# cristianpjensen/thesis-pai-reconstruction

Measured on NVIDIA B200. Metric: pix2pix_gan_train_images_per_sec_256x256, higher is better.
Workload: dtype bf16

## Files before the change

### thesis-pai-reconstruction_b200/csrc/igemm.cu

```cuda
#include <stdio.h>
#include <stdlib.h>

#include "pai_common.cuh"
#include "pai_epilogue.cuh"
#include "pai_kernels.h"

namespace pai {

#ifdef PAI_PROFILE_ROLES
#define ROLE_T0() const long long _t0 = clock64()
#define ROLE_ADD(var) var += clock64() - _t0
#else
#define ROLE_T0()
#define ROLE_ADD(var)
#endif

static constexpr int kThreads = 256;
static constexpr int kFpropThreads = 384;
static constexpr int kMaxStages = 8;

struct __align__(8) PipeSmem {
    uint64_t full[kMaxStages];
    uint64_t empty[kMaxStages];
    uint64_t acc_full[2];
// ... 315 lines not shown
            }
        };
        auto flush_stats = [&]() {
            if (st_col < 0) return;
            reduce_add(st_sum, st_sq, st_col);
#pragma unroll
            for (int j = 0; j < 8; ++j) st_sum[j] = st_sq[j] = 0.f;
            st_col = -1;
        };
        int it = 0;
        for (int t = worker; t < total_tiles; t += workers, ++it) {
            int nt, rr, mt, phase_idx, tw, th, tn;
            const int tt = p.fd_splitk.quot(t);
            p.fd_n_tiles.divmod(tt, rr, nt);
            p.fd_m_tiles.divmod(rr, phase_idx, mt);
            if (PAIR) mt = 2 * mt + (int)rank;
            p.fd_tiles_w.divmod(mt, mt, tw);
            p.fd_tiles_h.divmod(mt, tn, th);
            const int col0 = nt * n_tile;
            const int gw = tw * p.bw + (rpos & 255), gh = th * p.bh + ((rpos >> 8) & 255), gn = tn * p.bn + (rpos >> 16);
            const bool row_ok = (gw < p.gw) && (gh < p.gh) && (gn < p.gn);
            const int a = it & 1;
            const uint32_t acc_phase = (it >> 1) & 1;
            const bool fast = p.tma_out && (n_tile & 63) == 0 && col0 + n_tile <= p.cout &&
                              (p.bias == nullptr || (reinterpret_cast<uintptr_t>(p.bias) & 15) == 0);
            const int bw0 = tw * p.bw + (qpos & 255), bh0 = th * p.bh + ((qpos >> 8) & 255), bn0 = tn * p.bn + (qpos >> 16);
            const bool masked = MASKED && p.mask_src != nullptr && fast;
            auto mask_load = [&](int c) {
                __syncwarp();
                if (lane == 0) {
                    bulk_wait_group_read0();
                    mbar_expect_tx(&ps.mask_full[warp - 4], 32 * 128);
                    tma_load_4d(tile, &om.aux[fused ? c >> 6 : phase_idx], &ps.mask_full[warp - 4], col0 + (fused ? 0 : c),
                                bw0, bh0, bn0);
                }
            };
            if (masked && 64 * half < acc_n) mask_load(64 * half);
            {
                ROLE_T0();
                mbar_wait(&ps.acc_full[a], acc_phase);
                ROLE_ADD(prof_wait);
            }
#ifdef PAI_PROFILE_ROLES
            const long long twork = clock64();
#endif
            tc_fence_after();
            const uint32_t tmem_d = tmem_base + a * acc_cols + ((uint32_t)(q * 32) << 16);
// ... 64 lines not shown
                                if ((rows_ok >> row) & 1u) {
                                    const uint4 val = tile[row * 8 + (ch ^ (row & 7))];
                                    const __nv_bfloat162* hv = reinterpret_cast<const __nv_bfloat162*>(&val);
#pragma unroll
                                    for (int j = 0; j < 4; ++j) {
                                        const float2 f = __bfloat1622float2(hv[j]);
                                        cs[2 * j] += f.x;
                                        cs[2 * j + 1] += f.y;
                                        cq[2 * j] = fmaf(f.x, f.x, cq[2 * j]);
                                        cq[2 * j + 1] = fmaf(f.y, f.y, cq[2 * j + 1]);
                                    }
                                }
                            }
                            if (st_persist) {
#pragma unroll
                                for (int j = 0; j < 8; ++j) st_sum[j] += cs[j], st_sq[j] += cq[j];
                            } else {
                                reduce_add(cs, cq, col0 + oc);
                            }
                        }
                        if (masked && c + 128 < acc_n) mask_load(c + 128);
                    }
                }
            } else {
                const long long off = p.out_phase_off[phase_idx] + (long long)gn * p.out_sn + (long long)gh * p.out_sh +
                                      (long long)gw * p.out_sw + col0;
                const long long off2 = (long long)gn * p.out2_sn + (long long)gh * p.out2_sh + (long long)gw * p.out2_sw + col0;
                const bool vec_ok = ((p.cout & 7) == 0) && ((off & 7) == 0) && ((off2 & 7) == 0);
                int step = 0;
                for (int cc = 0; cc < n_tile; cc += 16, ++step) {
                    if ((step & 1) != half) continue;
                    uint32_t v[16];
                    __syncwarp();
                    tmem_ld_16(tmem_d + (uint32_t)cc, v);
                    tmem_ld_wait();
                    if (!row_ok || col0 + cc >= p.cout) continue;
                    float f[16];
#pragma unroll
                    for (int j = 0; j < 16; ++j) {
                        float x = __uint_as_float(v[j]);
                        if (p.bias != nullptr && col0 + cc + j < p.cout) x += __ldg(p.bias + col0 + cc + j);
                        f[j] = x;
                    }
                    if (p.accumulate) {
                        float* o = reinterpret_cast<float*>(p.out) + off + cc;
                        if (col0 + cc + 16 <= p.cout && ((off + cc) & 3) == 0) {
// ... 32 lines not shown
        if (p.bn_part != nullptr) flush_stats();
        if (lane == 0) bulk_wait_group0();
#ifdef PAI_PROFILE_ROLES
        if (blockIdx.x == 0 && threadIdx.x == 128)
            printf("[roles] epilogue warp 4: waiting for a full accumulator %lld cyc, working %lld cyc over %d tiles\n", prof_wait, prof_total, it);
#endif
    }
    tc_fence_before();
    if (PAIR)
        cluster_sync_all();
    else
        __syncthreads();
    if (warp == 2) {
        tc_fence_after();
        if (PAIR)
            tmem_dealloc_pair(tmem_base, 2 * acc_cols);
        else
            tmem_dealloc(tmem_base, 2 * acc_cols);
    }
}

__global__ void __launch_bounds__(kThreads, 1)
igemm_wgrad_kernel(const __grid_constant__ CUtensorMap tm_u, const __grid_constant__ CUtensorMap tm_s,
                   const IgemmWgradParams p) {
    pdl_launch_dependents();
    extern __shared__ uint8_t smem_raw[];
    __shared__ PipeSmem ps;
    uint8_t* smem = reinterpret_cast<uint8_t*>((reinterpret_cast<uintptr_t>(smem_raw) + 1023) & ~uintptr_t(1023));

    const int warp = threadIdx.x >> 5, lane = threadIdx.x & 31;
    const int mb = p.mb, nbt = p.nbt;
    const uint32_t blk_bytes = 64 * 128;
    const uint32_t a_bytes = 2 * mb * blk_bytes;
    const uint32_t stage_bytes = a_bytes + nbt * blk_bytes;
    const int stages = p.stages;
    const int n_cols = nbt * 64;
    const uint32_t tmem_cols = tmem_cols_for(mb * 256);

    const long long units = (long long)p.tiles * p.kblocks;
    const long long u_begin = units * blockIdx.x / gridDim.x, u_end = units * (blockIdx.x + 1) / gridDim.x;

    if (warp == 0 && lane == 0) {
        tma_prefetch_desc(&tm_u);
        tma_prefetch_desc(&tm_s);
    }
    if (warp == 1 && lane == 0) {
        for (int s = 0; s < stages; ++s) {
            mbar_init(&ps.full[s], 1);
            mbar_init(&ps.empty[s], 1);
        }
// ... 74 lines not shown
                    }
                }
                umma_commit(&ps.acc_full[0]);
                ++seg;
            }
        }
    } else if (warp >= 4) {
        const int q = warp & 3;
        const int r = q * 32 + lane;
        int seg = 0;
        long long u = u_begin;
        while (u < u_end) {
            const int tile = (int)(u / p.kblocks);
            const long long tile_end = (long long)(tile + 1) * p.kblocks;
            u = tile_end < u_end ? tile_end : u_end;
            const int ng = tile % p.n_groups, cu0 = (tile / p.n_groups) * 128 * mb;
            mbar_wait(&ps.acc_full[0], seg & 1);
            tc_fence_after();
            for (int a = 0; a < mb; ++a) {
                const int row = cu0 + a * 128 + r;
                const bool row_ok = row < p.cu;
                for (int nb = 0; nb < nbt; ++nb) {
                    const int blk = ng * nbt + nb, tap = blk / p.cs_blocks, cb = blk - tap * p.cs_blocks;
                    float* o = p.out + ((size_t)tap * p.cu + row) * (size_t)p.cs + cb * 64;
#pragma unroll
                    for (int c = 0; c < 64; c += 16) {
                        uint32_t v[16];
                        __syncwarp();
                        tmem_ld_16(tmem_base + ((uint32_t)(q * 32) << 16) + (uint32_t)(a * 256 + nb * 64 + c), v);
                        tmem_ld_wait();
                        if (row_ok) {
#pragma unroll
                            for (int j = 0; j < 16; j += 4)
                                red_add_v4(o + c + j, __uint_as_float(v[j]), __uint_as_float(v[j + 1]),
                                           __uint_as_float(v[j + 2]), __uint_as_float(v[j + 3]));
                        }
                    }
                }
            }
            tc_fence_before();
            __syncwarp();
            if (lane == 0) mbar_arrive_relaxed(&ps.acc_empty[0]);
            ++seg;
        }
    }
    tc_fence_before();
    __syncthreads();
    if (warp == 2) {
        tc_fence_after();
        tmem_dealloc(tmem_base, tmem_cols);
    }
}

static int pick_stages(size_t stage_bytes, size_t budget) {
    int s = (int)(budget / stage_bytes);
    if (s > kMaxStages) s = kMaxStages;
    if (s < 2) s = 2;
    return s;
}

bool igemm_fprop_use_pair(int n_tile, long long m_tiles, int n_tiles, int phases, int splitk) {
    static const bool off = getenv("PAI_NO_CTA_PAIR") != nullptr;
    if (off || splitk > 1 || n_tile % 32 != 0) return false;
    return ((m_tiles + 1) / 2) * n_tiles * phases >= 74;
}

int launch_igemm_fprop(const CUtensorMap& tm_a, const CUtensorMap& tm_b, const IgemmOutMaps& om, IgemmFpropParams p,
// ... 82 lines not shown
        const int c = (int)(i - pix * cout);
        float v = ws[i];
        if (bias != nullptr) v += bias[c];
        v = apply_act(v, act, slope);
        if (y_f32)
            reinterpret_cast<float*>(y)[pix * y_ld + c] = v;
        else
            reinterpret_cast<__nv_bfloat16*>(y)[pix * y_ld + c] = __float2bfloat16_rn(v);
    }
}

int launch_splitk_finish(const float* ws, long long pixels, int cout, const float* bias, int act, float slope, void* y,
                         int y_ld, int y_f32, cudaStream_t stream) {
    const long long total = pixels * cout;
    long long blocks = (total + 255) / 256;
    const int sms = sm_count(current_device());
    if (sms < 0) return -1;
    if (blocks > sms * 8) blocks = sms * 8;
    PAI_CUDA_OK(launch_pdl(splitk_finish_kernel, dim3((unsigned)blocks), dim3(256), 0, stream, 1, ws, total, cout, bias, act, slope, y, y_ld, y_f32));
    PAI_CUDA_OK(cudaGetLastError());
    return 0;
}

int launch_igemm_wgrad(const CUtensorMap& tm_u, const CUtensorMap& tm_s, IgemmWgradParams p, cudaStream_t stream) {
    const size_t stage_bytes = (size_t)(2 * p.mb + p.nbt) * 8192;
    p.stages = pick_stages(stage_bytes, 196 * 1024);
    const size_t smem = stage_bytes * p.stages + 1024;
    static DeviceOnce once;
    const int dev = current_device(), num_sms = persistent_ctas(dev);
    if (num_sms < 0) return -1;
    if (once.need(dev)) {
        PAI_CUDA_OK(cudaFuncSetAttribute(igemm_wgrad_kernel, cudaFuncAttributeMaxDynamicSharedMemorySize, 200 * 1024));
        once.mark(dev);
    }
    const long long units = (long long)p.tiles * p.kblocks;
    long long grid = units / 4 > p.tiles ? units / 4 : p.tiles;
    if (grid > num_sms) grid = num_sms;
    if (grid < 1) grid = 1;
    if (p.max_ctas > 0 && grid > p.max_ctas) grid = p.max_ctas;
    PAI_CUDA_OK(launch_pdl(igemm_wgrad_kernel, dim3((unsigned)grid), dim3(kThreads), smem, stream, 1, tm_u, tm_s, p));
    PAI_CUDA_OK(cudaGetLastError());
    return 0;
}

}
```

### thesis-pai-reconstruction_b200/csrc/pai_api.cu

```cuda
#include <stdarg.h>
#include <stdio.h>
#include <stdlib.h>
#include <string.h>

#include <cudaTypedefs.h>

#include "pai_common.cuh"
#include "pai_kernels.h"

namespace pai {

static thread_local char g_err[512] = "";

void set_error(const char* fmt, ...) {
    va_list ap;
    va_start(ap, fmt);
    vsnprintf(g_err, sizeof(g_err), fmt, ap);
    va_end(ap);
}

int cuda_fail(cudaError_t e, const char* what) {
    set_error("CUDA error %d (%s) at %s", (int)e, cudaGetErrorString(e), what);
    return -1;
}
// ... 29 lines not shown

static int g_reserved_sms = 0;

int persistent_ctas(int dev) {
    const int sms = sm_count(dev);
    if (sms < 0) return sms;
    int n = sms - __atomic_load_n(&g_reserved_sms, __ATOMIC_RELAXED);
    if (n < 2) n = 2;
    return n & ~1;
}

static PFN_cuTensorMapEncodeTiled_v12000 get_encode() {
    static PFN_cuTensorMapEncodeTiled_v12000 fn = nullptr;
    if (fn == nullptr) {
        void* p = nullptr;
        cudaDriverEntryPointQueryResult qres;
        if (cudaGetDriverEntryPoint("cuTensorMapEncodeTiled", &p, cudaEnableDefault, &qres) == cudaSuccess &&
            qres == cudaDriverEntryPointSuccess)
            fn = reinterpret_cast<PFN_cuTensorMapEncodeTiled_v12000>(p);
    }
    return fn;
}

int encode_tmap_bf16(CUtensorMap* map, const void* base, int rank, const uint64_t* dims,
                     const uint64_t* strides_bytes, const uint32_t* box) {
    auto fn = get_encode();
    PAI_REQUIRE(fn != nullptr, "cuTensorMapEncodeTiled driver entry point unavailable");
    cuuint32_t estr[5] = {1, 1, 1, 1, 1};
    CUresult r = fn(map, CU_TENSOR_MAP_DATA_TYPE_BFLOAT16, (cuuint32_t)rank, const_cast<void*>(base),
                    reinterpret_cast<const cuuint64_t*>(dims), reinterpret_cast<const cuuint64_t*>(strides_bytes),
                    reinterpret_cast<const cuuint32_t*>(box), estr, CU_TENSOR_MAP_INTERLEAVE_NONE,
                    CU_TENSOR_MAP_SWIZZLE_128B, CU_TENSOR_MAP_L2_PROMOTION_L2_256B,
                    CU_TENSOR_MAP_FLOAT_OOB_FILL_NONE);
    if (r != CUDA_SUCCESS) {
        set_error("cuTensorMapEncodeTiled failed (%d): rank %d dims [%llu %llu %llu %llu %llu] box [%u %u %u %u %u]",
                  (int)r, rank, (unsigned long long)dims[0], (unsigned long long)(rank > 1 ? dims[1] : 0),
                  (unsigned long long)(rank > 2 ? dims[2] : 0), (unsigned long long)(rank > 3 ? dims[3] : 0),
                  (unsigned long long)(rank > 4 ? dims[4] : 0), box[0], rank > 1 ? box[1] : 0, rank > 2 ? box[2] : 0,
                  rank > 3 ? box[3] : 0, rank > 4 ? box[4] : 0);
        return -3;
    }
    return 0;
}

static int pow2_ge(int v) {
    int p = 1;
    while (p < v) p <<= 1;
    return p;
}

struct PixBox {
    int bw, bh, bn, tiles_w, tiles_h, tiles_n;
};
static PixBox pick_box(int gw, int gh, int gn, int m) {
    PixBox b;
    b.bw = pow2_ge(gw) < m ? pow2_ge(gw) : m;
    int rest = m / b.bw;
    b.bh = pow2_ge(gh) < rest ? pow2_ge(gh) : rest;
    b.bn = rest / b.bh;
    b.tiles_w = (gw + b.bw - 1) / b.bw;
    b.tiles_h = (gh + b.bh - 1) / b.bh;
    b.tiles_n = (gn + b.bn - 1) / b.bn;
    return b;
}

static int map_unit(CUtensorMap* m, const void* base, int n, int h, int w, int c, int ld, const PixBox& b) {
    uint64_t dims[5] = {(uint64_t)c, (uint64_t)w, 1, (uint64_t)h, (uint64_t)n};
    uint64_t str[4] = {(uint64_t)ld * 2, (uint64_t)w * ld * 2, (uint64_t)w * ld * 2, (uint64_t)h * w * ld * 2};
    uint32_t box[5] = {64, (uint32_t)b.bw, 1, (uint32_t)b.bh, (uint32_t)b.bn};
    return encode_tmap_bf16(m, base, 5, dims, str, box);
}
static int map_split(CUtensorMap* m, const void* base, int n, int h, int w, int c, const PixBox& b) {
    uint64_t dims[5] = {(uint64_t)2 * c, (uint64_t)w / 2, 2, (uint64_t)h / 2, (uint64_t)n};
    uint64_t str[4] = {(uint64_t)2 * c * 2, (uint64_t)w * c * 2, (uint64_t)2 * w * c * 2, (uint64_t)h * w * c * 2};
    uint32_t box[5] = {64, (uint32_t)b.bw, 1, (uint32_t)b.bh, (uint32_t)b.bn};
    return encode_tmap_bf16(m, base, 5, dims, str, box);
}
static void s2_tap(int k, int* q, int* par) {
    static const int Q[4] = {-1, 0, 0, 1}, P[4] = {1, 0, 1, 0};
    *q = Q[k];
    *par = P[k];
}
static const int kTd[2][2] = {{0, -1}, {1, 0}};

static bool aligned16(const void* p) { return (reinterpret_cast<uintptr_t>(p) & 15) == 0; }

static int map_out(CUtensorMap* m, const void* base, int cout, int gw, int gh, int gn, long long sw, long long sh,
                   long long sn, const PixBox& b) {
    const int bw = b.bw < 32 ? b.bw : 32, bh = b.bh < 32 / bw ? b.bh : 32 / bw, bn = 32 / (bw * bh);
    if (sh == 0) sh = (long long)gw * sw;
    uint64_t dims[4] = {(uint64_t)cout, (uint64_t)gw, (uint64_t)gh, (uint64_t)gn};
    uint64_t str[3] = {(uint64_t)sw * 2, (uint64_t)sh * 2, (uint64_t)sn * 2};
    uint32_t box[4] = {64, (uint32_t)bw, (uint32_t)bh, (uint32_t)bn};
    return encode_tmap_bf16(m, base, 4, dims, str, box);
}

static int map_outputs(IgemmOutMaps* om, IgemmFpropParams& p, int nmaps, const PixBox& b) {
    p.tma_out = 0;
    const bool ok = !p.out_f32 && !p.accumulate && (p.cout & 7) == 0 && aligned16(p.out) && p.out_sw % 8 == 0 &&
                    p.out_sh % 8 == 0 && p.out_sn % 8 == 0 &&
                    (p.out2 == nullptr || (aligned16(p.out2) && p.out2_sw % 8 == 0 && p.out2_sh % 8 == 0 && p.out2_sn % 8 == 0));
    if (!ok) return 0;
    for (int j = 0; j < nmaps; ++j) {
        PAI_REQUIRE(p.out_phase_off[j] % 8 == 0, "igemm fprop: phase offset %lld is not 16 B aligned", p.out_phase_off[j]);
        int rc = map_out(&om->out[j], static_cast<const __nv_bfloat16*>(p.out) + p.out_phase_off[j], p.cout, p.gw, p.gh,
                         p.gn, p.out_sw, p.out_sh, p.out_sn, b);
        if (rc) return rc;
        if (p.mask_src != nullptr) {
            rc = map_out(&om->aux[j], static_cast<const __nv_bfloat16*>(p.mask_src) + p.out_phase_off[j], p.cout, p.gw,
                         p.gh, p.gn, p.out_sw, p.out_sh, p.out_sn, b);
            if (rc) return rc;
        }
    }
    if (p.out2 != nullptr) {
        int rc = map_out(&om->aux[0], p.out2, p.cout, p.gw, p.gh, p.gn, p.out2_sw, p.out2_sh, p.out2_sn, b);
        if (rc) return rc;
    }
    p.tma_out = 1;
    return 0;
}

static int auto_n_tile(int cout_pad, long long m_tiles_x_phases) {
    static const int cand[5] = {256, 128, 64, 32, 16};
    int best = 0;
    for (int i = 0; i < 5; ++i) {
        if (cout_pad % cand[i]) continue;
        if (best == 0) best = cand[i];
        if (m_tiles_x_phases * (cout_pad / cand[i]) >= 148) return cand[i];
        best = cand[i] >= 128 ? cand[i] : best;
        if (cand[i] <= 128) break;
    }
    return best;
}

static int pick_splitk(const void* ws, long long tiles, int num_kb) {
    if (ws == nullptr || tiles > 74 || num_kb < 8) return 1;
    long long s = 148 / tiles;
    if (s > num_kb / 2) s = num_kb / 2;
    return s < 2 ? 1 : (int)s;
}

}

using namespace pai;

extern "C" {

const char* pai_last_error(void) { return g_err; }
int pai_version(void) { return 100; }

int pai_reserve_sms(int n) {
    PAI_REQUIRE(n >= 0 && n <= 64, "pai_reserve_sms: reservation must be in 0..64 (got %d)", n);
    __atomic_store_n(&g_reserved_sms, n, __ATOMIC_RELAXED);
    return 0;
}

static int conv4x4_fprop_impl(const void* x, int n, int h, int w, int cin, int x_ld, const void* w_packed, int cout,
                              int cout_pad, int stride, const float* bias, int act, float slope, void* y, int y_ld,
// ... 36 lines not shown
    memset(&om, 0, sizeof(om));
    p.pair = pair;
    p.bw = b.bw, p.bh = b.bh, p.bn = b.bn, p.tiles_w = b.tiles_w, p.tiles_h = b.tiles_h;
    p.gw = wo, p.gh = ho, p.gn = n;
    p.n_tile = n_tile, p.cout = cout, p.kc_per_tap = cin / 64, p.ntaps = 16;
    for (int ky = 0; ky < 4; ++ky)
        for (int kx = 0; kx < 4; ++kx) {
            int t = ky * 4 + kx;
            if (stride == 2) {
                int qx, px, qy, py;
                s2_tap(kx, &qx, &px);
                s2_tap(ky, &qy, &py);
                p.tap_c[t] = px * cin, p.tap_w[t] = qx, p.tap_p[t] = py, p.tap_h[t] = qy;
            } else {
                p.tap_c[t] = 0, p.tap_w[t] = kx - 1, p.tap_p[t] = 0, p.tap_h[t] = ky - 1;
            }
        }
    p.b_rows_per_phase = cout_pad;
    p.bn_part = bn_part, p.bn_rows = bn_rows;
    p.splitk = splitk;
    if (p.splitk > 1) {
        p.out_sn = (long long)ho * wo * cout, p.out_sh = (long long)wo * cout, p.out_sw = cout;
        p.out_f32 = 1, p.accumulate = 1, p.out = splitk_ws;
        int rc2 = launch_igemm_fprop(tm_a, tm_b, om, p, m_tiles, cout_pad / n_tile, 1, (cudaStream_t)stream);
        if (rc2) return rc2;
        return launch_splitk_finish(splitk_ws, (long long)n * ho * wo, cout, bias, act, slope, y, y_ld, y_f32,
                                    (cudaStream_t)stream);
    }
    p.out_sn = (long long)ho * wo * y_ld, p.out_sh = (long long)wo * y_ld, p.out_sw = y_ld;
    p.bias = bias, p.act = act, p.slope = slope, p.out_f32 = y_f32, p.out = y;
    if (y2 != nullptr) {
        PAI_REQUIRE(!y_f32 && y2_ld % 8 == 0 && aligned16(y2) && aligned16(y) && y_ld % 8 == 0 && cout % 64 == 0,
                    "pai_conv4x4_fprop_dual: two bf16 outputs need cout %% 64 == 0 and 16 B aligned rows");
        p.out2 = y2, p.act2 = act2;
        p.out2_sn = (long long)ho * wo * y2_ld, p.out2_sh = (long long)wo * y2_ld, p.out2_sw = y2_ld;
    }
    rc = map_outputs(&om, p, 1, b);
    if (rc) return rc;
    return launch_igemm_fprop(tm_a, tm_b, om, p, m_tiles, cout_pad / n_tile, 1, (cudaStream_t)stream);
}

int pai_conv4x4_fprop_dual(const void* x, int n, int h, int w, int cin, int x_ld, const void* w_packed, int cout,
                           int cout_pad, int stride, const float* bias, int act, float slope, void* y, int y_ld, void* y2,
                           int y2_ld, int act2, int n_tile, void* stream) {
    PAI_REQUIRE(y2 != nullptr, "pai_conv4x4_fprop_dual: null second output");
    return conv4x4_fprop_impl(x, n, h, w, cin, x_ld, w_packed, cout, cout_pad, stride, bias, act, slope, y, y_ld, 0, n_tile,
                              nullptr, nullptr, 0, stream, y2, y2_ld, act2);
// ... 82 lines not shown
                    for (int ty = 0; ty < 2; ++ty)
                        for (int tx = 0; tx < 2; ++tx)
                            if (kTd[py][ty] == dy && kTd[px][tx] == dx) {
                                p.box_users[bi][nu] = ph * 4 + ty * 2 + tx;
                                p.box_col[bi][nu] = col;
                                ++nu;
                            }
                }
            p.box_nu[bi] = nu;
            bool consecutive = nu > 1;
            for (int u = 1; u < nu; ++u) consecutive = consecutive && p.box_col[bi][u] == p.box_col[bi][u - 1] + 1;
            p.box_merge[bi] = merge_ok && consecutive;
            for (; nu < 4; ++nu) p.box_users[bi][nu] = -1, p.box_col[bi][nu] = 0;
        }
        for (int py = 0; py < 2; ++py)
            for (int px = 0; px < 2; ++px) p.out_phase_off[col_of_phase[py * 2 + px]] = (py * wo + px) * ld;
        p.bias = bias, p.act = act, p.slope = slope, p.out_f32 = 0, p.out = y;
        rc = map_outputs(&om, p, 4, b);
        if (rc) return rc;
        return launch_igemm_fprop(tm_a, tm_b, om, p, m_tiles, 1, 1, (cudaStream_t)stream);
    }
    if (p.splitk > 1) {
        p.out_f32 = 1, p.accumulate = 1, p.out = splitk_ws;
        int rc2 = launch_igemm_fprop(tm_a, tm_b, om, p, m_tiles, cout_pad / n_tile, 4, (cudaStream_t)stream);
        if (rc2) return rc2;
        return launch_splitk_finish(splitk_ws, 4LL * n * h * w, cout, bias, act, slope, y, y_ld, y_f32,
                                    (cudaStream_t)stream);
    }
    p.bias = bias, p.act = act, p.slope = slope, p.out_f32 = y_f32, p.out = y;
    rc = map_outputs(&om, p, 4, b);
    if (rc) return rc;
    return launch_igemm_fprop(tm_a, tm_b, om, p, m_tiles, cout_pad / n_tile, 4, (cudaStream_t)stream);
}

int pai_convT4x4s2_fprop(const void* x, int n, int h, int w, int cin, int x_ld, const void* w_packed, int cout,
                         int cout_pad, const float* bias, int act, float slope, void* y, int y_ld, int y_f32,
                         int n_tile, float* splitk_ws, void* stream) {
    return convT4x4s2_fprop_impl(x, n, h, w, cin, x_ld, w_packed, cout, cout_pad, bias, act, slope, y, y_ld, y_f32, n_tile,
                                 splitk_ws, nullptr, 0, stream);
}
int pai_convT4x4s2_fprop_bnstats(const void* x, int n, int h, int w, int cin, int x_ld, const void* w_packed, int cout,
                                 int cout_pad, const float* bias, void* y, int y_ld, int n_tile, float* bn_partials,
                                 int bn_rows, void* stream) {
    PAI_REQUIRE(bn_partials != nullptr && bn_rows > 0, "pai_convT4x4s2_fprop_bnstats: null partial-sum buffer");
    return convT4x4s2_fprop_impl(x, n, h, w, cin, x_ld, w_packed, cout, cout_pad, bias, PAI_ACT_NONE, 0.f, y, y_ld, 0,
                                 n_tile, nullptr, bn_partials, bn_rows, stream);
}
// ... 33 lines not shown
    for (int ky = 0; ky < 4; ++ky)
        for (int kx = 0; kx < 4; ++kx) {
            int t = ky * 4 + kx;
            if (stride == 2) {
                int qx, px, qy, py;
                s2_tap(kx, &qx, &px);
                s2_tap(ky, &qy, &py);
                p.tap_c[t] = px * cs, p.tap_w[t] = qx, p.tap_p[t] = py, p.tap_h[t] = qy;
            } else if (stride == 1) {
                p.tap_c[t] = 0, p.tap_w[t] = kx - 1, p.tap_p[t] = 0, p.tap_h[t] = ky - 1;
            }
        }
    if (stride == 3)
        for (int t = 0; t < 9; ++t) p.tap_c[t] = 0, p.tap_w[t] = t % 3 - 1, p.tap_p[t] = 0, p.tap_h[t] = t / 3 - 1;
    const int ntaps = stride == 0 ? 1 : (stride == 3 ? 9 : 16);
    p.kblocks = b.tiles_w * b.tiles_h * b.tiles_n;
    p.cs_blocks = cs / 64;
    const int nb_total = ntaps * p.cs_blocks;
    p.nbt = nb_total % 4 == 0 ? 4 : (nb_total % 2 == 0 ? 2 : 1);
    p.n_groups = nb_total / p.nbt;
    p.mb = cu > 128 ? 2 : 1;
    p.tiles = ((cu + 128 * p.mb - 1) / (128 * p.mb)) * p.n_groups;
    p.max_ctas = splitk > 0 ? splitk * p.tiles : 0;
    return launch_igemm_wgrad(tm_u, tm_s, p, stream);
}

int pai_conv4x4_wgrad(const void* x, int n, int h, int w, int cin, int x_ld, const void* gy, int cout, int gy_ld,
                      int stride, float* dw, int splitk, void* stream) {
    PAI_REQUIRE(stride == 1 || stride == 2, "pai_conv4x4_wgrad: stride must be 1 or 2");
    const int ho = stride == 2 ? h / 2 : h - 1, wo = stride == 2 ? w / 2 : w - 1;
    return wgrad_common(gy, n, ho, wo, cout, gy_ld, x, h, w, cin, x_ld, stride, dw, splitk, (cudaStream_t)stream,
                        "pai_conv4x4_wgrad");
}

int pai_pointwise_wgrad(const void* u, long long m, int cu, int u_ld, const void* s, int cs, int s_ld, float* dw,
                        int splitk, void* stream) {
    PAI_REQUIRE(m > 0 && m < (1LL << 31), "pai_pointwise_wgrad: bad row count");
    return wgrad_common(u, 1, 1, (int)m, cu, u_ld, s, 1, (int)m, cs, s_ld, 0, dw, splitk, (cudaStream_t)stream,
                        "pai_pointwise_wgrad");
}

int pai_pointwise_gemm(const void* x, long long m, int cin, int x_ld, const void* w_packed, int cout, int cout_pad,
                       const float* bias, int act, float slope, void* y, int y_ld, int y_f32, void* y2, int y2_ld,
                       int act2, int n_tile, int k_valid, void* stream) {
    PAI_REQUIRE(x && w_packed && y, "pai_pointwise_gemm: null pointer");
    PAI_REQUIRE(k_valid == 0 || (cin == 64 && k_valid > 0 && k_valid <= 64 && k_valid % 16 == 0),
                "pai_pointwise_gemm: k_valid (%d) needs cin == 64 and a multiple of 16", k_valid);
// ... 51 lines not shown
                "pai_conv3x3_fprop: bad n_tile %d for cout_pad %d", n_tile, cout_pad);
    CUtensorMap tm_a, tm_b;
    int rc = map_unit(&tm_a, x, n, h, w, cin, x_ld, b);
    if (rc) return rc;
    uint64_t bd[2] = {(uint64_t)9 * cin, (uint64_t)cout_pad};
    uint64_t bs[1] = {(uint64_t)9 * cin * 2};
    uint32_t bb[2] = {64, (uint32_t)n_tile};
    rc = encode_tmap_bf16(&tm_b, w_packed, 2, bd, bs, bb);
    if (rc) return rc;
    IgemmFpropParams p;
    memset(&p, 0, sizeof(p));
    IgemmOutMaps om;
    memset(&om, 0, sizeof(om));
    p.bw = b.bw, p.bh = b.bh, p.bn = b.bn, p.tiles_w = b.tiles_w, p.tiles_h = b.tiles_h;
    p.gw = w, p.gh = h, p.gn = n;
    p.n_tile = n_tile, p.cout = cout, p.kc_per_tap = cin / 64, p.ntaps = 9;
    for (int t = 0; t < 9; ++t) p.tap_c[t] = 0, p.tap_w[t] = t % 3 - 1, p.tap_p[t] = 0, p.tap_h[t] = t / 3 - 1;
    p.b_rows_per_phase = cout_pad;
    const int m_tiles = b.tiles_w * b.tiles_h * b.tiles_n;
    p.splitk = pick_splitk(splitk_ws, (long long)m_tiles * (cout_pad / n_tile), 9 * (cin / 64));
    if (p.splitk > 1) {
        p.out_sn = (long long)h * w * cout, p.out_sh = (long long)w * cout, p.out_sw = cout;
        p.out_f32 = 1, p.accumulate = 1, p.out = splitk_ws;
        int rc2 = launch_igemm_fprop(tm_a, tm_b, om, p, m_tiles, cout_pad / n_tile, 1, (cudaStream_t)stream);
        if (rc2) return rc2;
        return launch_splitk_finish(splitk_ws, (long long)n * h * w, cout, bias, act, slope, y, y_ld, y_f32,
                                    (cudaStream_t)stream);
    }
    p.out_sn = (long long)h * w * y_ld, p.out_sh = (long long)w * y_ld, p.out_sw = y_ld;
    p.bias = bias, p.act = act, p.slope = slope, p.out_f32 = y_f32, p.out = y;
    rc = map_outputs(&om, p, 1, b);
    if (rc) return rc;
    return launch_igemm_fprop(tm_a, tm_b, om, p, m_tiles, cout_pad / n_tile, 1, (cudaStream_t)stream);
}

int pai_conv3x3_wgrad(const void* x, int n, int h, int w, int cin, int x_ld, const void* gy, int cout, int gy_ld,
                      float* dw, void* stream) {
    return wgrad_common(gy, n, h, w, cout, gy_ld, x, h, w, cin, x_ld, 3, dw, 0, (cudaStream_t)stream,
                        "pai_conv3x3_wgrad");
}

}
```

### thesis-pai-reconstruction_b200/csrc/pai_common.cuh

```cuda
#pragma once
#include <cuda.h>
#include <cuda_bf16.h>
#include <cuda_runtime.h>
#include <stdint.h>
#include <stdio.h>

namespace pai {

void set_error(const char* fmt, ...);
int cuda_fail(cudaError_t e, const char* what);
#define PAI_CUDA_OK(expr)                                                   \
    do {                                                                    \
        cudaError_t _e = (expr);                                            \
        if (_e != cudaSuccess) return ::pai::cuda_fail(_e, #expr);          \
    } while (0)
#define PAI_REQUIRE(cond, ...)                                              \
    do {                                                                    \
        if (!(cond)) {                                                      \
            ::pai::set_error(__VA_ARGS__);                                  \
            return -2;                                                      \
        }                                                                   \
    } while (0)

struct DeviceOnce {
// ... 11 lines not shown
template <typename... KArgs, typename... Args>
static inline cudaError_t launch_pdl(void (*kernel)(KArgs...), dim3 grid, dim3 block, size_t smem, cudaStream_t st,
                                     int cluster_x, Args&&... args) {
    cudaLaunchConfig_t cfg = {};
    cfg.gridDim = grid, cfg.blockDim = block, cfg.dynamicSmemBytes = smem, cfg.stream = st;
    cudaLaunchAttribute attr[2];
    int na = 0;
    if (cluster_x > 1) {
        attr[na].id = cudaLaunchAttributeClusterDimension;
        attr[na].val.clusterDim.x = (unsigned)cluster_x, attr[na].val.clusterDim.y = 1, attr[na].val.clusterDim.z = 1;
        ++na;
    }
    if (pdl_enabled()) {
        attr[na].id = cudaLaunchAttributeProgrammaticStreamSerialization;
        attr[na].val.programmaticStreamSerializationAllowed = 1;
        ++na;
    }
    cfg.attrs = attr, cfg.numAttrs = (unsigned)na;
    return cudaLaunchKernelEx(&cfg, kernel, static_cast<KArgs>(args)...);
}

int encode_tmap_bf16(CUtensorMap* map, const void* base, int rank, const uint64_t* dims,
                     const uint64_t* strides_bytes , const uint32_t* box);

#ifdef __CUDACC__
__device__ __forceinline__ uint32_t smem_u32(const void* p) {
    return static_cast<uint32_t>(__cvta_generic_to_shared(p));
}

__device__ __forceinline__ bool elect_one() {
    uint32_t pred;
    asm volatile(
        "{\n"
        ".reg .pred P;\n"
        "elect.sync _|P, 0xffffffff;\n"
        "selp.u32 %0, 1, 0, P;\n"
        "}\n"
        : "=r"(pred));
    return pred != 0;
}

__device__ __forceinline__ void mbar_init(uint64_t* bar, uint32_t count) {
    asm volatile("mbarrier.init.shared::cta.b64 [%0], %1;" ::"r"(smem_u32(bar)), "r"(count) : "memory");
}
__device__ __forceinline__ void mbar_fence_init() {
    asm volatile("fence.mbarrier_init.release.cluster;" ::: "memory");
// ... 41 lines not shown
    asm volatile(
        "cp.async.bulk.tensor.5d.shared::cluster.global.mbarrier::complete_tx::bytes [%0], [%1, {%3, %4, %5, %6, "
        "%7}], [%2];" ::"r"(smem_u32(dst)),
        "l"(reinterpret_cast<uint64_t>(map)), "r"(smem_u32(bar)), "r"(c0), "r"(c1), "r"(c2), "r"(c3), "r"(c4)
        : "memory");
}
__device__ __forceinline__ void tma_prefetch_5d(const CUtensorMap* map, int c0, int c1, int c2, int c3, int c4) {
    asm volatile("cp.async.bulk.prefetch.tensor.5d.L2.global.tile [%0, {%1, %2, %3, %4, %5}];" ::"l"(
                     reinterpret_cast<uint64_t>(map)),
                 "r"(c0), "r"(c1), "r"(c2), "r"(c3), "r"(c4)
                 : "memory");
}
__device__ __forceinline__ void tma_load_4d(void* dst, const CUtensorMap* map, uint64_t* bar, int c0, int c1, int c2,
                                            int c3) {
    asm volatile(
        "cp.async.bulk.tensor.4d.shared::cluster.global.mbarrier::complete_tx::bytes [%0], [%1, {%3, %4, %5, %6}], [%2];"
        ::"r"(smem_u32(dst)), "l"(reinterpret_cast<uint64_t>(map)), "r"(smem_u32(bar)), "r"(c0), "r"(c1), "r"(c2), "r"(c3)
        : "memory");
}
__device__ __forceinline__ void tma_store_4d(const CUtensorMap* map, const void* src, int c0, int c1, int c2, int c3) {
    asm volatile("cp.async.bulk.tensor.4d.global.shared::cta.bulk_group [%0, {%2, %3, %4, %5}], [%1];" ::"l"(
                     reinterpret_cast<uint64_t>(map)),
                 "r"(smem_u32(src)), "r"(c0), "r"(c1), "r"(c2), "r"(c3)
                 : "memory");
}
__device__ __forceinline__ void bulk_commit_group() { asm volatile("cp.async.bulk.commit_group;" ::: "memory"); }
__device__ __forceinline__ void bulk_wait_group_read0() { asm volatile("cp.async.bulk.wait_group.read 0;" ::: "memory"); }
__device__ __forceinline__ void bulk_wait_group0() { asm volatile("cp.async.bulk.wait_group 0;" ::: "memory"); }
__device__ __forceinline__ void tma_prefetch_desc(const CUtensorMap* map) {
    asm volatile("prefetch.tensormap [%0];" ::"l"(reinterpret_cast<uint64_t>(map)) : "memory");
}

__device__ __forceinline__ void tmem_alloc(uint32_t* dst_smem, uint32_t ncols) {
    asm volatile("tcgen05.alloc.cta_group::1.sync.aligned.shared::cta.b32 [%0], %1;" ::"r"(smem_u32(dst_smem)),
                 "r"(ncols)
                 : "memory");
    asm volatile("tcgen05.relinquish_alloc_permit.cta_group::1.sync.aligned;" ::: "memory");
}
__device__ __forceinline__ void tmem_dealloc(uint32_t taddr, uint32_t ncols) {
    asm volatile("tcgen05.dealloc.cta_group::1.sync.aligned.b32 %0, %1;" ::"r"(taddr), "r"(ncols) : "memory");
}
__device__ __forceinline__ void tc_fence_before() { asm volatile("tcgen05.fence::before_thread_sync;" ::: "memory"); }
__device__ __forceinline__ void tc_fence_after() { asm volatile("tcgen05.fence::after_thread_sync;" ::: "memory"); }

__device__ __forceinline__ void umma_bf16_ss(uint32_t tmem_d, uint64_t desc_a, uint64_t desc_b, uint32_t idesc,
                                             uint32_t accumulate) {
// ... 198 lines not shown
```

### thesis-pai-reconstruction_b200/csrc/pai_kernels.h

```cpp
#pragma once
#include <cuda.h>
#include <cuda_runtime.h>
#include <stdint.h>

#include "../../include/pai_b200.h"

namespace pai {

struct FastDiv {
    uint32_t mul, shift, div;
#ifdef __CUDACC__
    __device__ __forceinline__ int quot(int n) const { return (int)((__umulhi((uint32_t)n, mul) + (uint32_t)n) >> shift); }
    __device__ __forceinline__ void divmod(int n, int& q, int& r) const {
        q = quot(n);
        r = n - q * (int)div;
    }
#endif
};
inline FastDiv make_fastdiv(int d) {
    FastDiv f;
    f.div = (uint32_t)d;
    uint32_t s = 0;
    while ((1u << s) < (uint32_t)d) ++s;
    f.shift = s;
// ... 39 lines not shown
    int accumulate;
    int tma_out;
};

struct IgemmOutMaps {
    CUtensorMap out[4];
    CUtensorMap aux[4];
};

struct IgemmWgradParams {
    int bw, bh, bn;
    int tiles_w, tiles_h, tiles_n;
    int kblocks;
    int mb;
    int nbt;
    int cs_blocks;
    int n_groups;
    int tiles;
    int max_ctas;
    int cu, cs;
    int stages;
    int tap_c[16], tap_w[16], tap_p[16], tap_h[16];
    float* out;
};

bool igemm_fprop_use_pair(int n_tile, long long m_tiles, int n_tiles, int phases, int splitk);
int launch_igemm_fprop(const CUtensorMap& tm_a, const CUtensorMap& tm_b, const IgemmOutMaps& om, IgemmFpropParams p,
                       int m_tiles, int n_tiles, int phases, cudaStream_t stream);
int launch_splitk_finish(const float* ws, long long pixels, int cout, const float* bias, int act, float slope, void* y,
                         int y_ld, int y_f32, cudaStream_t stream);
int launch_igemm_wgrad(const CUtensorMap& tm_u, const CUtensorMap& tm_s, IgemmWgradParams p, cudaStream_t stream);

}
```

Baseline: 9293.

## Use TMA bulk reduce-add for split-K fprop and wgrad fp32 accumulation

Split-K fprop and wgrad epilogues now stage fp32 accumulator chunks in swizzled shared memory and issue TMA cp.reduce.async.bulk add operations into global fp32 tensors. Previously they used per-thread atomic or scalar global accumulation. The wgrad launcher also gains a cost model that may pick a grid aligned to the tile count, to cut the number of partial-tile flushes. Along with the new fp32 tensor maps and env switches, this adds shared-memory staging buffers and per-chunk bulk-group waits that could serialize the epilogue.

Result: faster. 9489 (median of 6 runs) (+2.1%).

```diff
diff --git a/thesis-pai-reconstruction_b200/csrc/igemm.cu b/thesis-pai-reconstruction_b200/csrc/igemm.cu
--- a/thesis-pai-reconstruction_b200/csrc/igemm.cu
+++ b/thesis-pai-reconstruction_b200/csrc/igemm.cu
@@ -361,7 +361,8 @@
             const bool row_ok = (gw < p.gw) && (gh < p.gh) && (gn < p.gn);
             const int a = it & 1;
             const uint32_t acc_phase = (it >> 1) & 1;
-            const bool fast = p.tma_out && (n_tile & 63) == 0 && col0 + n_tile <= p.cout &&
+            const bool red = !PAIR && !MASKED && p.accumulate && p.tma_out;
+            const bool fast = !p.accumulate && p.tma_out && (n_tile & 63) == 0 && col0 + n_tile <= p.cout &&
                               (p.bias == nullptr || (reinterpret_cast<uintptr_t>(p.bias) & 15) == 0);
             const int bw0 = tw * p.bw + (qpos & 255), bh0 = th * p.bh + ((qpos >> 8) & 255), bn0 = tn * p.bn + (qpos >> 16);
             const bool masked = MASKED && p.mask_src != nullptr && fast;
@@ -472,6 +473,27 @@
                         if (masked && c + 128 < acc_n) mask_load(c + 128);
                     }
                 }
+            } else if (red) {
+                int step = 0;
+                for (int c = 0; c < n_tile; c += 32, ++step) {
+                    if ((step & 1) != half) continue;
+                    uint32_t v[32];
+                    tmem_ld_16(tmem_d + (uint32_t)c, *reinterpret_cast<uint32_t(*)[16]>(&v[0]));
+                    tmem_ld_16(tmem_d + (uint32_t)(c + 16), *reinterpret_cast<uint32_t(*)[16]>(&v[16]));
+                    tmem_ld_wait();
+                    if (c + 64 >= n_tile) release_acc();
+                    if (lane == 0) bulk_wait_group_read0();
+                    __syncwarp();
+#pragma unroll
+                    for (int j = 0; j < 8; ++j)
+                        tile[lane * 8 + (j ^ (lane & 7))] = make_uint4(v[4 * j], v[4 * j + 1], v[4 * j + 2], v[4 * j + 3]);
+                    fence_proxy_async_smem();
+                    __syncwarp();
+                    if (lane == 0) {
+                        tma_reduce_add_4d(&om.out[phase_idx], tile, col0 + c, bw0, bh0, bn0);
+                        bulk_commit_group();
+                    }
+                }
             } else {
                 const long long off = p.out_phase_off[phase_idx] + (long long)gn * p.out_sn + (long long)gh * p.out_sh +
                                       (long long)gw * p.out_sw + col0;
@@ -550,10 +572,11 @@
 
 __global__ void __launch_bounds__(kThreads, 1)
 igemm_wgrad_kernel(const __grid_constant__ CUtensorMap tm_u, const __grid_constant__ CUtensorMap tm_s,
-                   const IgemmWgradParams p) {
+                   const __grid_constant__ CUtensorMap tm_out, const IgemmWgradParams p) {
     pdl_launch_dependents();
     extern __shared__ uint8_t smem_raw[];
     __shared__ PipeSmem ps;
+    __shared__ __align__(1024) uint4 stage_buf[4][32 * 8];
     uint8_t* smem = reinterpret_cast<uint8_t*>((reinterpret_cast<uintptr_t>(smem_raw) + 1023) & ~uintptr_t(1023));
 
     const int warp = threadIdx.x >> 5, lane = threadIdx.x & 31;
@@ -674,6 +697,29 @@
                 const bool row_ok = row < p.cu;
                 for (int nb = 0; nb < nbt; ++nb) {
                     const int blk = ng * nbt + nb, tap = blk / p.cs_blocks, cb = blk - tap * p.cs_blocks;
+                    if (p.tma_out) {
+                        uint4* tile = stage_buf[q];
+                        for (int c = 0; c < 64; c += 32) {
+                            uint32_t v[32];
+                            const uint32_t taddr = tmem_base + ((uint32_t)(q * 32) << 16) + (uint32_t)(a * 256 + nb * 64 + c);
+                            __syncwarp();
+                            tmem_ld_16(taddr, *reinterpret_cast<uint32_t(*)[16]>(&v[0]));
+                            tmem_ld_16(taddr + 16, *reinterpret_cast<uint32_t(*)[16]>(&v[16]));
+                            tmem_ld_wait();
+                            if (lane == 0) bulk_wait_group_read0();
+                            __syncwarp();
+#pragma unroll
+                            for (int j = 0; j < 8; ++j)
+                                tile[lane * 8 + (j ^ (lane & 7))] = make_uint4(v[4 * j], v[4 * j + 1], v[4 * j + 2], v[4 * j + 3]);
+                            fence_proxy_async_smem();
+                            __syncwarp();
+                            if (lane == 0) {
+                                tma_reduce_add_3d(&tm_out, tile, cb * 64 + c, cu0 + a * 128 + q * 32, tap);
+                                bulk_commit_group();
+                            }
+                        }
+                        continue;
+                    }
                     float* o = p.out + ((size_t)tap * p.cu + row) * (size_t)p.cs + cb * 64;
 #pragma unroll
                     for (int c = 0; c < 64; c += 16) {
@@ -695,6 +741,7 @@
             if (lane == 0) mbar_arrive_relaxed(&ps.acc_empty[0]);
             ++seg;
         }
+        if (lane == 0) bulk_wait_group0();
     }
     tc_fence_before();
     __syncthreads();
@@ -823,7 +870,8 @@
     return 0;
 }
 
-int launch_igemm_wgrad(const CUtensorMap& tm_u, const CUtensorMap& tm_s, IgemmWgradParams p, cudaStream_t stream) {
+int launch_igemm_wgrad(const CUtensorMap& tm_u, const CUtensorMap& tm_s, const CUtensorMap& tm_out, IgemmWgradParams p,
+                       cudaStream_t stream) {
     const size_t stage_bytes = (size_t)(2 * p.mb + p.nbt) * 8192;
     p.stages = pick_stages(stage_bytes, 196 * 1024);
     const size_t smem = stage_bytes * p.stages + 1024;
@@ -839,7 +887,21 @@
     if (grid > num_sms) grid = num_sms;
     if (grid < 1) grid = 1;
     if (p.max_ctas > 0 && grid > p.max_ctas) grid = p.max_ctas;
-    PAI_CUDA_OK(launch_pdl(igemm_wgrad_kernel, dim3((unsigned)grid), dim3(kThreads), smem, stream, 1, tm_u, tm_s, p));
+    if (p.max_ctas == 0 && p.tiles < grid) {
+        const long long aligned = grid / p.tiles * p.tiles;
+        const double unit_us = 2.0 * 128 * p.mb * 64 * p.nbt * 64 / 15e6;
+        const double flush_us = 128.0 * p.mb * 64 * p.nbt * 4 / 2e6;
+        auto cost = [&](long long g) {
+            long long segs = 0;
+            for (long long b = 0; b < g; ++b) {
+                const long long u0 = units * b / g, u1 = units * (b + 1) / g;
+                if (u1 > u0) segs += (u1 - 1) / p.kblocks - u0 / p.kblocks + 1;
+            }
+            return (double)((units + g - 1) / g) * unit_us + (double)segs * flush_us;
+        };
+        if (cost(aligned) < cost(grid)) grid = aligned;
+    }
+    PAI_CUDA_OK(launch_pdl(igemm_wgrad_kernel, dim3((unsigned)grid), dim3(kThreads), smem, stream, 1, tm_u, tm_s, tm_out, p));
     PAI_CUDA_OK(cudaGetLastError());
     return 0;
 }
diff --git a/thesis-pai-reconstruction_b200/csrc/pai_api.cu b/thesis-pai-reconstruction_b200/csrc/pai_api.cu
--- a/thesis-pai-reconstruction_b200/csrc/pai_api.cu
+++ b/thesis-pai-reconstruction_b200/csrc/pai_api.cu
@@ -75,12 +75,12 @@
     return fn;
 }
 
-int encode_tmap_bf16(CUtensorMap* map, const void* base, int rank, const uint64_t* dims,
-                     const uint64_t* strides_bytes, const uint32_t* box) {
+static int encode_tmap(CUtensorMap* map, CUtensorMapDataType dtype, const void* base, int rank, const uint64_t* dims,
+                       const uint64_t* strides_bytes, const uint32_t* box) {
     auto fn = get_encode();
     PAI_REQUIRE(fn != nullptr, "cuTensorMapEncodeTiled driver entry point unavailable");
     cuuint32_t estr[5] = {1, 1, 1, 1, 1};
-    CUresult r = fn(map, CU_TENSOR_MAP_DATA_TYPE_BFLOAT16, (cuuint32_t)rank, const_cast<void*>(base),
+    CUresult r = fn(map, dtype, (cuuint32_t)rank, const_cast<void*>(base),
                     reinterpret_cast<const cuuint64_t*>(dims), reinterpret_cast<const cuuint64_t*>(strides_bytes),
                     reinterpret_cast<const cuuint32_t*>(box), estr, CU_TENSOR_MAP_INTERLEAVE_NONE,
                     CU_TENSOR_MAP_SWIZZLE_128B, CU_TENSOR_MAP_L2_PROMOTION_L2_256B,
@@ -94,6 +94,14 @@
         return -3;
     }
     return 0;
+}
+int encode_tmap_bf16(CUtensorMap* map, const void* base, int rank, const uint64_t* dims, const uint64_t* strides_bytes,
+                     const uint32_t* box) {
+    return encode_tmap(map, CU_TENSOR_MAP_DATA_TYPE_BFLOAT16, base, rank, dims, strides_bytes, box);
+}
+int encode_tmap_f32(CUtensorMap* map, const void* base, int rank, const uint64_t* dims, const uint64_t* strides_bytes,
+                    const uint32_t* box) {
+    return encode_tmap(map, CU_TENSOR_MAP_DATA_TYPE_FLOAT32, base, rank, dims, strides_bytes, box);
 }
 
 static int pow2_ge(int v) {
@@ -139,13 +147,33 @@
 static bool aligned16(const void* p) { return (reinterpret_cast<uintptr_t>(p) & 15) == 0; }
 
 static int map_out(CUtensorMap* m, const void* base, int cout, int gw, int gh, int gn, long long sw, long long sh,
-                   long long sn, const PixBox& b) {
+                   long long sn, const PixBox& b, bool f32 = false) {
     const int bw = b.bw < 32 ? b.bw : 32, bh = b.bh < 32 / bw ? b.bh : 32 / bw, bn = 32 / (bw * bh);
+    const int es = f32 ? 4 : 2;
     if (sh == 0) sh = (long long)gw * sw;
     uint64_t dims[4] = {(uint64_t)cout, (uint64_t)gw, (uint64_t)gh, (uint64_t)gn};
-    uint64_t str[3] = {(uint64_t)sw * 2, (uint64_t)sh * 2, (uint64_t)sn * 2};
-    uint32_t box[4] = {64, (uint32_t)bw, (uint32_t)bh, (uint32_t)bn};
-    return encode_tmap_bf16(m, base, 4, dims, str, box);
+    uint64_t str[3] = {(uint64_t)sw * es, (uint64_t)sh * es, (uint64_t)sn * es};
+    uint32_t box[4] = {(uint32_t)(128 / es), (uint32_t)bw, (uint32_t)bh, (uint32_t)bn};
+    return f32 ? encode_tmap_f32(m, base, 4, dims, str, box) : encode_tmap_bf16(m, base, 4, dims, str, box);
+}
+
+static bool tma_reduce_off() {
+    static const bool off = getenv("PAI_NO_TMA_REDUCE") != nullptr;
+    return off;
+}
+
+static int map_workspace(IgemmOutMaps* om, IgemmFpropParams& p, int nmaps, const PixBox& b) {
+    p.tma_out = 0;
+    if (tma_reduce_off() || (p.cout & 3) != 0 || (p.n_tile & 31) != 0 || !aligned16(p.out)) return 0;
+    for (int j = 0; j < nmaps; ++j)
+        if (p.out_phase_off[j] % 4 != 0) return 0;
+    for (int j = 0; j < nmaps; ++j) {
+        int rc = map_out(&om->out[j], static_cast<const float*>(p.out) + p.out_phase_off[j], p.cout, p.gw, p.gh, p.gn,
+                         p.out_sw, p.out_sh, p.out_sn, b, true);
+        if (rc) return rc;
+    }
+    p.tma_out = 1;
+    return 0;
 }
 
 static int map_outputs(IgemmOutMaps* om, IgemmFpropParams& p, int nmaps, const PixBox& b) {
@@ -187,6 +215,8 @@
 }
 
 static int pick_splitk(const void* ws, long long tiles, int num_kb) {
+    static const int forced = getenv("PAI_SPLITK_FORCE") ? atoi(getenv("PAI_SPLITK_FORCE")) : 0;
+    if (ws != nullptr && forced > 0) return forced < num_kb ? forced : num_kb;
     if (ws == nullptr || tiles > 74 || num_kb < 8) return 1;
     long long s = 148 / tiles;
     if (s > num_kb / 2) s = num_kb / 2;
@@ -269,7 +299,9 @@
     if (p.splitk > 1) {
         p.out_sn = (long long)ho * wo * cout, p.out_sh = (long long)wo * cout, p.out_sw = cout;
         p.out_f32 = 1, p.accumulate = 1, p.out = splitk_ws;
-        int rc2 = launch_igemm_fprop(tm_a, tm_b, om, p, m_tiles, cout_pad / n_tile, 1, (cudaStream_t)stream);
+        int rc2 = map_workspace(&om, p, 1, b);
+        if (rc2) return rc2;
+        rc2 = launch_igemm_fprop(tm_a, tm_b, om, p, m_tiles, cout_pad / n_tile, 1, (cudaStream_t)stream);
         if (rc2) return rc2;
         return launch_splitk_finish(splitk_ws, (long long)n * ho * wo, cout, bias, act, slope, y, y_ld, y_f32,
                                     (cudaStream_t)stream);
@@ -398,7 +430,9 @@
     }
     if (p.splitk > 1) {
         p.out_f32 = 1, p.accumulate = 1, p.out = splitk_ws;
-        int rc2 = launch_igemm_fprop(tm_a, tm_b, om, p, m_tiles, cout_pad / n_tile, 4, (cudaStream_t)stream);
+        int rc2 = map_workspace(&om, p, 4, b);
+        if (rc2) return rc2;
+        rc2 = launch_igemm_fprop(tm_a, tm_b, om, p, m_tiles, cout_pad / n_tile, 4, (cudaStream_t)stream);
         if (rc2) return rc2;
         return launch_splitk_finish(splitk_ws, 4LL * n * h * w, cout, bias, act, slope, y, y_ld, y_f32,
                                     (cudaStream_t)stream);
@@ -478,7 +512,17 @@
     p.mb = cu > 128 ? 2 : 1;
     p.tiles = ((cu + 128 * p.mb - 1) / (128 * p.mb)) * p.n_groups;
     p.max_ctas = splitk > 0 ? splitk * p.tiles : 0;
-    return launch_igemm_wgrad(tm_u, tm_s, p, stream);
+    CUtensorMap tm_out;
+    memset(&tm_out, 0, sizeof(tm_out));
+    p.tma_out = !tma_reduce_off() && aligned16(dw);
+    if (p.tma_out) {
+        uint64_t dims[3] = {(uint64_t)cs, (uint64_t)cu, (uint64_t)ntaps};
+        uint64_t str[2] = {(uint64_t)cs * 4, (uint64_t)cu * cs * 4};
+        uint32_t box[3] = {32, 32, 1};
+        rc = encode_tmap_f32(&tm_out, dw, 3, dims, str, box);
+        if (rc) return rc;
+    }
+    return launch_igemm_wgrad(tm_u, tm_s, tm_out, p, stream);
 }
 
 int pai_conv4x4_wgrad(const void* x, int n, int h, int w, int cin, int x_ld, const void* gy, int cout, int gy_ld,
@@ -576,7 +620,9 @@
     if (p.splitk > 1) {
         p.out_sn = (long long)h * w * cout, p.out_sh = (long long)w * cout, p.out_sw = cout;
         p.out_f32 = 1, p.accumulate = 1, p.out = splitk_ws;
-        int rc2 = launch_igemm_fprop(tm_a, tm_b, om, p, m_tiles, cout_pad / n_tile, 1, (cudaStream_t)stream);
+        int rc2 = map_workspace(&om, p, 1, b);
+        if (rc2) return rc2;
+        rc2 = launch_igemm_fprop(tm_a, tm_b, om, p, m_tiles, cout_pad / n_tile, 1, (cudaStream_t)stream);
         if (rc2) return rc2;
         return launch_splitk_finish(splitk_ws, (long long)n * h * w, cout, bias, act, slope, y, y_ld, y_f32,
                                     (cudaStream_t)stream);
diff --git a/thesis-pai-reconstruction_b200/csrc/pai_common.cuh b/thesis-pai-reconstruction_b200/csrc/pai_common.cuh
--- a/thesis-pai-reconstruction_b200/csrc/pai_common.cuh
+++ b/thesis-pai-reconstruction_b200/csrc/pai_common.cuh
@@ -57,6 +57,8 @@
 
 int encode_tmap_bf16(CUtensorMap* map, const void* base, int rank, const uint64_t* dims,
                      const uint64_t* strides_bytes , const uint32_t* box);
+int encode_tmap_f32(CUtensorMap* map, const void* base, int rank, const uint64_t* dims,
+                    const uint64_t* strides_bytes , const uint32_t* box);
 
 #ifdef __CUDACC__
 __device__ __forceinline__ uint32_t smem_u32(const void* p) {
@@ -144,6 +146,18 @@
     asm volatile("cp.async.bulk.tensor.4d.global.shared::cta.bulk_group [%0, {%2, %3, %4, %5}], [%1];" ::"l"(
                      reinterpret_cast<uint64_t>(map)),
                  "r"(smem_u32(src)), "r"(c0), "r"(c1), "r"(c2), "r"(c3)
+                 : "memory");
+}
+__device__ __forceinline__ void tma_reduce_add_4d(const CUtensorMap* map, const void* src, int c0, int c1, int c2, int c3) {
+    asm volatile("cp.reduce.async.bulk.tensor.4d.global.shared::cta.add.tile.bulk_group [%0, {%2, %3, %4, %5}], [%1];" ::"l"(
+                     reinterpret_cast<uint64_t>(map)),
+                 "r"(smem_u32(src)), "r"(c0), "r"(c1), "r"(c2), "r"(c3)
+                 : "memory");
+}
+__device__ __forceinline__ void tma_reduce_add_3d(const CUtensorMap* map, const void* src, int c0, int c1, int c2) {
+    asm volatile("cp.reduce.async.bulk.tensor.3d.global.shared::cta.add.tile.bulk_group [%0, {%2, %3, %4}], [%1];" ::"l"(
+                     reinterpret_cast<uint64_t>(map)),
+                 "r"(smem_u32(src)), "r"(c0), "r"(c1), "r"(c2)
                  : "memory");
 }
 __device__ __forceinline__ void bulk_commit_group() { asm volatile("cp.async.bulk.commit_group;" ::: "memory"); }
diff --git a/thesis-pai-reconstruction_b200/csrc/pai_kernels.h b/thesis-pai-reconstruction_b200/csrc/pai_kernels.h
--- a/thesis-pai-reconstruction_b200/csrc/pai_kernels.h
+++ b/thesis-pai-reconstruction_b200/csrc/pai_kernels.h
@@ -85,6 +85,7 @@
     int stages;
     int tap_c[16], tap_w[16], tap_p[16], tap_h[16];
     float* out;
+    int tma_out;
 };
 
 bool igemm_fprop_use_pair(int n_tile, long long m_tiles, int n_tiles, int phases, int splitk);
@@ -92,6 +93,7 @@
                        int m_tiles, int n_tiles, int phases, cudaStream_t stream);
 int launch_splitk_finish(const float* ws, long long pixels, int cout, const float* bias, int act, float slope, void* y,
                          int y_ld, int y_f32, cudaStream_t stream);
-int launch_igemm_wgrad(const CUtensorMap& tm_u, const CUtensorMap& tm_s, IgemmWgradParams p, cudaStream_t stream);
+int launch_igemm_wgrad(const CUtensorMap& tm_u, const CUtensorMap& tm_s, const CUtensorMap& tm_out, IgemmWgradParams p,
+                       cudaStream_t stream);
 
 }
```
